# tud-amr/multi-robot-fabrics

Hardware: NVIDIA B200
Metric: fabric robot-steps/sec (3 Panda RF-CV) (higher is better)
Workload: dtype f32

## Files before the change

### __graft_entry__.py

```python
from __future__ import annotations

import os
import subprocess
import sys

ROOT = os.path.dirname(os.path.abspath(__file__))
PKG = os.path.join(ROOT, "multi-robot-fabrics_b200")
NVCC_FLAGS = ["-gencode", "arch=compute_100a,code=sm_100a", "-lineinfo", "-O3", "-std=c++17",
              "-Xcompiler", "-fPIC", "-shared"]


def _newer(target: str, sources) -> bool:
    if not os.path.exists(target):
        return False
    t = os.path.getmtime(target)
    return all(os.path.getmtime(s) <= t for s in sources)


def build(force: bool = False) -> None:
    csrc = os.path.join(PKG, "csrc")
    srcs = [os.path.join(csrc, f) for f in ("mrf_b200.cu", "mrf_device.cuh", "mrf_devcfg.h", "mrf_coop.cuh")]
    srcs.append(os.path.join(ROOT, "include", "mrf_b200.h"))
    so = os.path.join(PKG, "libmrf_b200.so")
    if force or not _newer(so, srcs):
        nvcc = os.environ.get("NVCC", "nvcc")
        subprocess.check_call([nvcc, *NVCC_FLAGS, "-o", so, srcs[0]])
    subprocess.check_call(["make", "-C", os.path.join(ROOT, "oracle"), "-s"])
    emul_so = os.path.join(ROOT, "tests", "emul", "libmrf_emul.so")
    emul_src = os.path.join(ROOT, "tests", "emul", "mrf_emul.cpp")
    if force or not _newer(emul_so, srcs[1:] + [emul_src]):
        subprocess.check_call(["g++", "-O2", "-std=c++17", "-fPIC", "-shared", "-ffp-contract=off", "-o", emul_so,
                               emul_src])
    if ROOT not in sys.path:
        sys.path.insert(0, ROOT)
    _probe_reference()
    import multi_robot_fabrics_b200 as m

    m._lib.lib()
    for name in m._lib.EXPORTS:
        getattr(m._lib.lib(), name)


_PROBED = False


def _probe_reference() -> None:
    global _PROBED
    if _PROBED:
        return
    _PROBED = True
    import importlib.util
    ref = os.path.join(ROOT, "baseline", "_ref")
    if os.path.isdir(ref) and ref not in sys.path:
        sys.path.append(ref)
    spec = importlib.util.spec_from_file_location("make_reference_golden",
                                                  os.path.join(ROOT, "tests", "golden", "make_reference_golden.py"))
    mod = importlib.util.module_from_spec(spec)
    spec.loader.exec_module(mod)
    ok, msg = mod.probe()
    gold = os.path.join(ROOT, "tests", "golden", "reference_golden.npz")
    state = "present" if os.path.exists(gold) else "absent"
    if ok:
        print(f"[build] reference dependencies available ({msg}); reference_golden.npz {state} -- "
              f"`python tests/golden/make_reference_golden.py` (re)generates it", file=sys.stderr)
    else:
        print(f"[build] reference dependencies {msg}: fabric arithmetic stays parity-unpinned "
              f"(baseline/_ref {'exists' if os.path.isdir(ref) else 'does not exist'}; reference_golden.npz {state})", file=sys.stderr)


def smoke() -> None:
    if ROOT not in sys.path:
        sys.path.insert(0, ROOT)
    import numpy as np
    import torch

    import multi_robot_fabrics_b200 as m
    from multi_robot_fabrics_b200.api import Fabrics, to_soa
    from oracle import o2
    from oracle.deadlock_ref import DeadlockOracle

    R, N, dev = 3, 20, "cuda:0"
    fab = Fabrics(R, device=0, estimate_goal=1, dl_dist_endeff=1.0)
    ocfg = o2.default_config(R)

    rec = m.scenarios.generate(64, R, seed=123)
# ... 80 lines not shown
```

### multi-robot-fabrics_b200/csrc/mrf_b200.cu

```cuda
#include <cuda_runtime.h>

#include <cmath>
#include <cstdio>
#include <cstdlib>
#include <cstring>
#include <new>
#include <string>
#include <vector>

#include "../../include/mrf_b200.h"
#include "mrf_device.cuh"
#include "mrf_devcfg.h"
#include "mrf_coop.cuh"

namespace mrf {

struct DlCfg {
    long long g_sr, g_sc, w_sr;
    int est_robot;
    int R, time_wait, time_gate;
    double avg_vel_constant, dist_constant, w_follower, w_leader, goal_scale, dist_endeff, backoff;
};

__device__ __forceinline__ double np_norm3(double x, double y, double z) {
// ... 281 lines not shown
            const unsigned t = atomicAdd(&sync[0], 1u);
            while (*reinterpret_cast<volatile unsigned*>(&sync[1]) + window <= t) __nanosleep(100);
            *tk = t;
        }
        __syncthreads();
        tile = *tk;
    }
    const long long b = (long long)tile * kTile + lane;
    const bool live = b < Bn;
    const long long bb = live ? b : Bn - 1;
    const T* ld_base = rec + (long long)r * B + bb;
    long long ld_stride = (long long)R * B;
    const T* tail = rec_tail;
    if (AOS) {
        const long long first = (long long)tile * kTile;
        const int nb = (int)(B - first < kTile ? B - first : kTile);
        const int nvals = nb * R * n_var;
        const int nvec = nvals * (int)sizeof(T) / 16;
        const T* srcT = rec + first * R * n_var;
        const int4* src = reinterpret_cast<const int4*>(srcT);
        int4* dst = reinterpret_cast<int4*>(kin);
        for (int i = tid; i < nvec; i += NT) dst[i] = src[i];
        for (int i = nvec * (16 / (int)sizeof(T)) + tid; i < nvals; i += NT) kin[i] = srcT[i];
        __syncthreads();
        if (tid == 0) atomicAdd(&sync[1], 1u);
        ld_base = kin + ((live ? lane : nb - 1) * R + r) * n_var;
        ld_stride = 1;
        tail += r * MRF_REC;
    }
    const long long b_src = STRIDE ? (long long)ex.list[bb] : 0;
    auto ld = [&](int f) {
        if (STRIDE)
            return f < ex.src_nvar ? (T)ex.src[f * ex.sf + r * ex.sr + b_src * ex.sb] : (T)ex.src_tail[r * MRF_REC + f];
        return AOS ? (f < n_var ? ld_base[f] : tail[f]) : rec[((long long)f * R + r) * B + bb];
    };
    (void)ld_stride;

    T q[kDof], qd[kDof];
#pragma unroll
    for (int i = 0; i < kDof; ++i) {
        q[i] = ld(MRF_Q + i);
        qd[i] = ld(MRF_QD + i);
    }
    load_params<T>(ld, prm, NT, tid);
    T* st_sph = prm + P_N * NT;
    if (!UNIFORM && !AOS && n_static > 0) {
        for (int i = 0; i < 4 * n_static; ++i) st_sph[i * NT + tid] = ex.stat[((long long)i * R + r) * B + bb];
    }
    if (AOS && ex.rec_out != nullptr && live) {
        for (int f = 0; f < n_var; ++f) ex.rec_out[((long long)f * R + r) * B + b] = ld_base[f];
    }
    Chain<T> ch;
    const T vref = cfg.static_or_dyn ? T(1) : T(0), aref = cfg.static_or_dyn ? cfg.sref : T(0);
    T acc = T(0);
    prm[P_RISK * NT + tid] = T(0);
    const bool want_pre = x_ee != nullptr || goal_est != nullptr || cfg.estimate_goal != 0;
    for (int k = want_pre ? -1 : 0; k < N; ++k) {
        if (k >= 0) {
#pragma unroll
            for (int i = 0; i < kDof; ++i) q[i] += cfg.dt * qd[i];
        }
        MRF_STEP_SYNC();
        chain_forward(cfg, r, q, qd, ch, kin, NT, tid);
        if (k < 0) {
            V3<T> p8 = kin_load(kin, NT, tid, 4, 0);
            if (x_ee != nullptr && live) {
                T* o = rec_order_out ? x_ee + (b * R + r) * 3 : x_ee + (long long)r * 3 * B + b;
                const long long st = rec_order_out ? 1 : B;
                o[0] = p8.x;
                o[st] = p8.y;
                o[2 * st] = p8.z;
            }
            if (r == cfg.estimate_robot) {
                V3<T> g = mk(prm[(P_G0 + 0) * NT + tid], prm[(P_G0 + 1) * NT + tid], prm[(P_G0 + 2) * NT + tid]);
                if (cfg.estimate_goal) {
                    V3<T> l1 = mk(cfg.link1[r][0], cfg.link1[r][1], cfg.link1[r][2]);
                    V3<T> v = cfg.estimate_goal == 1 ? cross(ch.z[0], p8 - l1) : kin_load(kin, NT, tid, 4, 3);
                    g = p8 + v * cfg.est_h;
                    prm[(P_G0 + 0) * NT + tid] = g.x;
                    prm[(P_G0 + 1) * NT + tid] = g.y;
                    prm[(P_G0 + 2) * NT + tid] = g.z;
                }
                if (goal_est != nullptr && live) {
                    T* o = rec_order_out ? goal_est + b * 3 : goal_est + b;
                    const long long st = rec_order_out ? 1 : B;
                    o[0] = g.x;
                    o[st] = g.y;
                    o[2 * st] = g.z;
                }
            }
            continue;
        }
        MRF_STEP_SYNC();
        T act[kDof], stiff;
        if (UNIFORM) {
            SmemSrcUniform<T, R> src{kin, lane, r, vref, aref, cfg.r_obst};
            fabric_action(cfg, r, q, qd, ch, kin, prm, NT, tid, src, act, &stiff);
        } else {
            SmemSrc<T> src{cfg, kin, NT, lane, r, vref, aref, st_sph, AOS ? 0 : n_static, tid};
            fabric_action(cfg, r, q, qd, ch, kin, prm, NT, tid, src, act, &stiff);
        }
        prm[P_RISK * NT + tid] = Mth<T>::max(prm[P_RISK * NT + tid], stiff);
#pragma unroll
        for (int i = 0; i < kDof; ++i) {
            qd[i] = act[i];
            acc += act[i] * act[i];
        }
        if (qN != nullptr && live) {
#pragma unroll
            for (int i = 0; i < kDof; ++i) qN[(((long long)r * N + k) * kDof + i) * B + b] = q[i];
        }
        if (qdN != nullptr && live) {
#pragma unroll
            for (int i = 0; i < kDof; ++i) qdN[(((long long)r * N + k) * kDof + i) * B + b] = qd[i];
        }
    }
    if (avg_vel != nullptr && live) avg_vel[rec_order_out ? b * R + r : (long long)r * B + b] = acc / (T(N) * T(kDof));
    if (risk != nullptr && live) risk[rec_order_out ? b * R + r : (long long)r * B + b] = prm[P_RISK * NT + tid];
    if (STRIDE) {
        __syncthreads();
        if (fused_post && tid < kTile && live)
            deadlock_one<float>(ex.dl.c, (long long)ex.list[b], ex.dl.B, (int)b, ex.dl.ov, ex.dl.x_ee, ex.dl.goals, ex.dl.weights,
                                ex.dl.avg_vel, nullptr, ex.dl.sm_state, ex.dl.time_step, ex.dl.tdo, ex.dl.st_int, ex.dl.st_goal,
                                ex.dl.flag, ex.dl.goal_est, ex.dl.result);
        tile_first += gridDim.x;
    }
    has_work = STRIDE && (long long)tile_first * kTile < Bn;
  }
    if (fused_post) {
        __syncthreads();
        if (threadIdx.x == 0) {
            __threadfence();
            if (atomicAdd(ex.dl.done, 1u) == gridDim.x - 1) {
                *ex.dl.done = 0;
                n_live[0] = 0;
            }
        }
    }
}

constexpr int kActThreads = 128;

#ifndef MRF_ACTION_MINBLOCKS
#define MRF_ACTION_MINBLOCKS 1
#endif
template <typename T, bool CART>
__global__ void __launch_bounds__(kActThreads, sizeof(T) == 4 ? MRF_ACTION_MINBLOCKS : 1)
    action_kernel(const __grid_constant__ DevCfg<T> cfg, int robot_first, int n_rob, const T* __restrict__ rec, int S,
                  const T* __restrict__ obst, int N, T* __restrict__ out, T* __restrict__ qN, T* __restrict__ qdN,
                  long long B, const int32_t* __restrict__ sm_state) {
// ... 615 lines not shown
extern "C" int mrf_set_coop_max_batch(mrf_handle_t h, int64_t max_batch) {
    if (!h || max_batch < 0) return fail(MRF_EINVAL, "mrf_set_coop_max_batch: bad argument");
    h->coop_max_batch = max_batch;
    return MRF_OK;
}
extern "C" int64_t mrf_launch_count(mrf_handle_t h) { return h ? h->launches : 0; }
extern "C" double mrf_last_kernel_ms(mrf_handle_t h) { return h ? h->last_ms : 0.0; }

template <typename T> static const DevCfg<T>& devcfg(mrf_handle_t h);
template <> const DevCfg<float>& devcfg<float>(mrf_handle_t h) { return h->c32; }
template <> const DevCfg<double>& devcfg<double>(mrf_handle_t h) { return h->c64; }

template <typename K> static int set_smem(K kernel, size_t bytes) {
    if (bytes > 48 * 1024) MRF_CUDA(cudaFuncSetAttribute(kernel, cudaFuncAttributeMaxDynamicSharedMemorySize, (int)bytes));
    return MRF_OK;
}
template <typename K> static void same_carveout(K kernel) {
#ifndef MRF_NO_CARVEOUT
    cudaFuncSetAttribute(kernel, cudaFuncAttributePreferredSharedMemoryCarveout, cudaSharedmemCarveoutMaxShared);
#endif
}

template <typename T>
static int rollout_dev(mrf_handle_t h, const T* rec, int N, T* avg_vel, T* x_ee, T* goal_est, T* qN, T* qdN, int64_t B,
                       void* stream, bool aos = false, int sync_slot = 0, int n_var = MRF_REC, const T* rec_tail = nullptr,
                       T* risk = nullptr, RollExtra<T> ex = RollExtra<T>{}) {
    unsigned* const n_live = ex.n_live;
    const int n_static = ex.n_static;
    const T* const stat = ex.stat;
    if (!h || (!rec && !n_live)) return fail(MRF_EINVAL, "mrf_rollout: null argument");
    if (B <= 0 || N <= 0) return fail(MRF_EINVAL, "mrf_rollout: B and N must be positive");
    MRF_CUDA(cudaSetDevice(h->device));
    const int R = h->cfg.n_robots, NT = kTile * R;
    if (aos && (qN || qdN)) return fail(MRF_EINVAL, "mrf_rollout: record-order input has no trajectory output");
    if (n_static < 0 || n_static > MRF_MAX_STATIC || (n_static > 0 && (!stat || aos || n_live)))
        return fail(MRF_EINVAL, "mrf_rollout: bad static-obstacle arguments");
    if (!aos && R >= 2 && B <= h->coop_max_batch && !risk && !n_live && n_static == 0) {
        switch (R) {
            case 2: rollout_coop_kernel<T, 2><<<(unsigned)B, 64, 0, (cudaStream_t)stream>>>(devcfg<T>(h), rec, N, avg_vel, x_ee, goal_est, qN, qdN, (long long)B); break;
            case 3: rollout_coop_kernel<T, 3><<<(unsigned)B, 96, 0, (cudaStream_t)stream>>>(devcfg<T>(h), rec, N, avg_vel, x_ee, goal_est, qN, qdN, (long long)B); break;
            case 4: rollout_coop_kernel<T, 4><<<(unsigned)B, 128, 0, (cudaStream_t)stream>>>(devcfg<T>(h), rec, N, avg_vel, x_ee, goal_est, qN, qdN, (long long)B); break;
            default: return fail(MRF_EINVAL, "mrf_rollout: n_robots out of range");
        }
        MRF_CUDA(cudaGetLastError());
        h->launches += 1;
        return MRF_OK;
    }
    const size_t smem = sizeof(T) * (size_t)(kKinRows<T> + P_N + 4 * n_static) * NT;
    long long grid = (B + kTile - 1) / kTile;
    if (n_live != nullptr && grid > 16) grid = 16;
    int rc = MRF_OK;
#define MRF_LAUNCH_ROLLOUT_K(RR, UU, AA, SS)                                                                         \
    {                                                                                                                \
        rc = set_smem(rollout_kernel<T, RR, UU, AA, SS>, smem);                                                      \
        same_carveout(rollout_kernel<T, RR, UU, AA, SS>);                                                            \
        if (rc) return rc;                                                                                           \
        rollout_kernel<T, RR, UU, AA, SS><<<(unsigned)grid, NT, smem, (cudaStream_t)stream>>>(                       \
            devcfg<T>(h), rec, N, avg_vel, x_ee, goal_est, qN, qdN, (long long)B, h->d_sync + 2 * sync_slot,        \
            (unsigned)h->zc_window, n_var, rec_tail, risk, ex);                                                      \
    }
#define MRF_LAUNCH_ROLLOUT(RR)                                                                                       \
    case RR:                                                                                                         \
        if (devcfg<T>(h).uniform_obst && n_static == 0) {                                                            \
            if (aos) MRF_LAUNCH_ROLLOUT_K(RR, true, true, false)                                                     \
            else if (stride) MRF_LAUNCH_ROLLOUT_STRIDE(RR, true)                                                     \
            else MRF_LAUNCH_ROLLOUT_K(RR, true, false, false)                                                        \
        } else {                                                                                                     \
            if (aos) MRF_LAUNCH_ROLLOUT_K(RR, false, true, false)                                                    \
            else if (stride) MRF_LAUNCH_ROLLOUT_STRIDE(RR, false)                                                    \
            else MRF_LAUNCH_ROLLOUT_K(RR, false, false, false)                                                       \
        }                                                                                                            \
        break;
#define MRF_LAUNCH_ROLLOUT_STRIDE(RR, UU)                                                                            \
    {                                                                                                                \
        if constexpr (sizeof(T) == 8) MRF_LAUNCH_ROLLOUT_K(RR, UU, false, true)                                      \
        else return fail(MRF_EINVAL, "mrf_rollout: device-side count is FP64 only");                                 \
    }
    const bool stride = n_live != nullptr;
    if (aos) MRF_CUDA(cudaMemsetAsync(h->d_sync + 2 * sync_slot, 0, 2 * sizeof(unsigned), (cudaStream_t)stream));
    switch (R) {
        MRF_LAUNCH_ROLLOUT(1)
        MRF_LAUNCH_ROLLOUT(2)
        MRF_LAUNCH_ROLLOUT(3)
        MRF_LAUNCH_ROLLOUT(4)
        default: return fail(MRF_EINVAL, "mrf_rollout: n_robots out of range");
    }
#undef MRF_LAUNCH_ROLLOUT_STRIDE
#undef MRF_LAUNCH_ROLLOUT_K
#undef MRF_LAUNCH_ROLLOUT
    MRF_CUDA(cudaGetLastError());
    h->launches += 1;
    return MRF_OK;
}

template <typename T, bool CART>
static int action_dev(mrf_handle_t h, int robot_first, int n_rob, const T* rec, int S, const T* obst, int N, T* out,
                      T* qN, T* qdN, int64_t B, void* stream, const int32_t* sm_state = nullptr) {
    if (!h || !rec || (S > 0 && !obst)) return fail(MRF_EINVAL, "mrf_action: null argument");
    if (B <= 0 || S < 0 || n_rob < 1 || robot_first < 0 || robot_first + n_rob > h->cfg.n_robots)
        return fail(MRF_EINVAL, "mrf_action: bad sizes");
    if (CART && N <= 0) return fail(MRF_EINVAL, "mrf_rollout_cart: needs N > 0");
    MRF_CUDA(cudaSetDevice(h->device));
    static const int env_thr = getenv("MRF_ACTION_THREADS_F64") ? atoi(getenv("MRF_ACTION_THREADS_F64")) : 32;
    const int threads = sizeof(T) == 8 ? env_thr : kActThreads;
    const size_t smem = sizeof(T) * (size_t)(kKinRows<T> + P_N + kObstRing * MRF_OBST) * threads;
    int rc = set_smem(action_kernel<T, CART>, smem);
    if (rc) return rc;
    const long long total = (long long)n_rob * B;
    const long long grid = (total + threads - 1) / threads;
    action_kernel<T, CART><<<(unsigned)grid, threads, smem, (cudaStream_t)stream>>>(
// ... 1274 lines not shown
```

### multi-robot-fabrics_b200/csrc/mrf_device.cuh

```cuda
#pragma once

#include <stdint.h>

#if defined(__CUDACC__)
#define MRF_HD __host__ __device__ __forceinline__
#else
#define MRF_HD inline
#include <cmath>
#endif

#include "../../include/mrf_b200.h"

namespace mrf {

template <int N> struct Int {
    static constexpr int value = N;
};

constexpr int kDof = 7;
constexpr int kEgo = 5;
constexpr int kPts = kEgo + 1;
constexpr int kZ = kPts * 9;
#ifdef MRF_AXES_SMEM_F32
template <typename T> constexpr bool kAxesInSmem = true;
// ... 419 lines not shown
    V3<P2<T>> b;
    V3<P2<T>> nv;
};
template <typename T> MRF_HD void acc2_zero(PointAcc2<T>& a) {
    const P2<T> z = psplat(T(0));
    a.A = Sym3<P2<T>>{z, z, z, z, z, z};
    a.b = V3<P2<T>>{z, z, z};
    a.nv = V3<P2<T>>{z, z, z};
}
template <typename T, bool IRHO>
MRF_HD void sphere_leaf2(const V3<P2<T>>& p, const V3<P2<T>>& v, const V3<P2<T>>& cc, const V3<P2<T>>& xo,
                         const V3<P2<T>>& vo, const V3<P2<T>>& co, T vref, T aref, P2<T> rho, P2<T> irho, P2<T> cM, T sigma,
                         PointAcc2<T>& acc) {
    const P2<T> m1 = psplat(T(-1)), nvref = psplat(-vref);
    V3<P2<T>> d{pfma(xo.x, m1, p.x), pfma(xo.y, m1, p.y), pfma(xo.z, m1, p.z)};
    V3<P2<T>> w{pfma(vo.x, nvref, v.x), pfma(vo.y, nvref, v.y), pfma(vo.z, nvref, v.z)};
    P2<T> n2 = pdot(d, d);
    P2<T> in1 = prsqrt(n2);
    P2<T> gs, ix, nrin;
    if (IRHO) {
        gs = pmul(in1, irho);
        ix = prcp(pfma(n2, gs, m1));
        nrin = pmul(in1, rho);
    } else {
        P2<T> n = pmul(n2, in1);
        P2<T> t = pfma(rho, m1, n);
        P2<T> nr = pmul(n, rho);
        P2<T> u = prcp(pmul(nr, t));
        gs = pmul(u, t);
        ix = pmul(pmul(u, nr), rho);
        nrin = pmul(pmul(in1, rho), m1);
    }
    P2<T> dw = pdot(d, w), da = pdot(d, co);
    P2<T> wc = pfma(d.z, cc.z, pfma(d.y, cc.y, pfma(d.x, cc.x, pdot(w, w))));
    P2<T> ix2 = pmul(ix, ix), ix4 = pmul(ix2, ix2);
    P2<T> Ml = pmul(cM, ix4);
    P2<T> Mg = pmul(Ml, gs);
    P2<T> k = pmul(Mg, gs);
    P2<T> u1 = pmul(k, pmul(dw, dw));
    P2<T> hh = pmul(ix4, psplat(T(-0.5)));
    P2<T> fl = pmul(u1, hh);
    P2<T> fd = pmul(u1, pfma(ix, psplat(T(2)), hh));
    P2<T> X = pfma(u1, nrin, pmul(Mg, wc));
    P2<T> fq = pfma(X, psplat(sigma), pfma(pmul(Mg, da), psplat(-aref), fl));
    P2<T> ge = pmul(gs, pfma(X, psplat(sigma - T(1)), fd));
    acc.nv.x = pfma(d.x, ge, acc.nv.x); acc.nv.y = pfma(d.y, ge, acc.nv.y); acc.nv.z = pfma(d.z, ge, acc.nv.z);
    V3<P2<T>> Md{pmul(d.x, k), pmul(d.y, k), pmul(d.z, k)};
    acc.A.xx = pfma(Md.x, d.x, acc.A.xx); acc.A.xy = pfma(Md.x, d.y, acc.A.xy); acc.A.xz = pfma(Md.x, d.z, acc.A.xz);
    acc.A.yy = pfma(Md.y, d.y, acc.A.yy); acc.A.yz = pfma(Md.y, d.z, acc.A.yz); acc.A.zz = pfma(Md.z, d.z, acc.A.zz);
    P2<T> gf = pmul(gs, fq);
    acc.b.x = pfma(d.x, gf, acc.b.x); acc.b.y = pfma(d.y, gf, acc.b.y); acc.b.z = pfma(d.z, gf, acc.b.z);
}

template <typename T>
MRF_HD void plane_leaf(V3<T> p, V3<T> v, V3<T> cc, V3<T> nh, T dn, T rb, T wt, T sigma, PointAcc<T>& acc, T& num) {
    T x = dot(nh, p) + dn - rb;
    T xd = dot(nh, v);
    T s = xd > T(0) ? T(0) : (xd < T(0) ? T(1) : T(0.5));
    T ix = Mth<T>::rcp(x);
    T xd2 = xd * xd;
    T Ml = ((T(0.2) * wt) * s) * ix * ix;
    T u = Ml * xd2;
    T h = T(-10) * xd2 * Mth<T>::rcp(T(1) + Mth<T>::exp(T(10) * x));
    T fl = Ml * h;
    T X = Ml * dot(nh, cc);
    T fq = fl + sigma * X;
    num += xd * ((fl + u * ix) + (sigma - T(1)) * X);
    V3<T> Mg = nh * Ml;
    acc.A.xx += Mg.x * nh.x; acc.A.xy += Mg.x * nh.y; acc.A.xz += Mg.x * nh.z;
    acc.A.yy += Mg.y * nh.y; acc.A.yz += Mg.y * nh.z; acc.A.zz += Mg.z * nh.z;
    acc.b = acc.b + nh * fq;
}

template <typename T, int K, typename Org>
MRF_HD void jac_cols(const Chain<T>& ch, const T* kin, int NT, int tid, V3<T> p, const Org& org, V3<T>* Jc) {
#pragma unroll
    for (int j = 0; j < K; ++j) Jc[j] = cross(axis_of(ch, kin, NT, tid, j), p - org(j));
}

template <typename T, int K> MRF_HD void pullback(const V3<T>* Jc, const PointAcc<T>& acc, Spec<T>& S) {
#pragma unroll
    for (int j = 0; j < K; ++j) {
        V3<T> AJ = symmul(acc.A, Jc[j]);
        S.f[j] += dot(Jc[j], acc.b);
#pragma unroll
        for (int i = 0; i <= j; ++i) S.M[i][j] += dot(Jc[i], AJ);
    }
}

template <typename T> MRF_HD void chol_solve6(T (&M)[6][6], T eps, const T* b, T* x) {
    T inv[6];
#pragma unroll
    for (int j = 0; j < 6; ++j) {
        T s = M[j][j] + eps;
#pragma unroll
        for (int k = 0; k < j; ++k) s -= M[k][j] * M[k][j];
        T r = Mth<T>::rsqrt(s);
        inv[j] = r;
        M[j][j] = s * r;
#pragma unroll
        for (int i = j + 1; i < 6; ++i) {
            T t = M[j][i];
#pragma unroll
            for (int k = 0; k < j; ++k) t -= M[k][j] * M[k][i];
            M[j][i] = t * r;
        }
// ... 75 lines not shown
        for (int k = 0; k < i; ++k) s += N[k][i] * y[k];
        y[i] = s * inv[i];
    }
#pragma unroll
    for (int i = 5; i >= 0; --i) {
        T s = y[i];
#pragma unroll
        for (int k = i + 1; k < 6; ++k) s += N[i][k] * x[k];
        x[i] = s * inv[i];
    }
}
template <typename T> MRF_HD void chol_solve6n_pair(P2<T> (&N)[6][6], T eps, const P2<T>* b, P2<T>* x) {
    P2<T> inv[6];
    const P2<T> ne = psplat(-eps);
#pragma unroll
    for (int j = 0; j < 6; ++j) {
        P2<T> s = padd(N[j][j], ne);
#pragma unroll
        for (int k = 0; k < j; ++k) s = pfma(N[k][j], N[k][j], s);
        P2<T> r = pmk(Mth<T>::rsqrt(-plo(s)), Mth<T>::rsqrt(-phi(s)));
        inv[j] = r;
#pragma unroll
        for (int i = j + 1; i < 6; ++i) {
            P2<T> t = N[j][i];
#pragma unroll
            for (int k = 0; k < j; ++k) t = pfma(N[k][j], N[k][i], t);
            N[j][i] = pmul(t, r);
        }
    }
    P2<T> y[6];
#pragma unroll
    for (int i = 0; i < 6; ++i) {
        P2<T> s = b[i];
#pragma unroll
        for (int k = 0; k < i; ++k) s = pfma(N[k][i], y[k], s);
        y[i] = pmul(s, inv[i]);
    }
#pragma unroll
    for (int i = 5; i >= 0; --i) {
        P2<T> s = y[i];
#pragma unroll
        for (int k = i + 1; k < 6; ++k) s = pfma(N[i][k], x[k], s);
        x[i] = pmul(s, inv[i]);
    }
}

template <typename T> MRF_HD void attractor_scalars(T n, T w, T& dpsi, T& m2) {
    dpsi = T(5) * w * Mth<T>::tanh(T(10) * n);
    m2 = T(2) * (T(1.7) * Mth<T>::exp(T(-0.5625) * n * n) + T(0.3));
}

template <typename T, typename Src>
MRF_HD void fabric_action(const DevCfg<T>& cfg, int r, const T* q, const T* qd, const Chain<T>& ch, const T* kin,
                          const T* prm, int NT, int tid, const Src& src, T* act, T* stiff = nullptr) {
    const T sigma = cfg.sigma;
    T stiff_sum = T(0);
    Spec<T> G;
#pragma unroll
    for (int i = 0; i < 6; ++i) {
#pragma unroll
        for (int j = 0; j < 6; ++j) G.M[i][j] = T(0);
        G.M[i][i] = T(-0.2);
        G.f[i] = T(0);
    }
    G.m7 = T(0.2);
    G.f[6] = T(0);
    T num = T(0);

#pragma unroll
    for (int i = 0; i < kDof; ++i) {
        const P2<T> x2 = pmk(q[i] - cfg.lim[i][0], cfg.lim[i][1] - q[i]);
        const T sl = qd[i] > T(0) ? T(0) : (qd[i] < T(0) ? T(1) : T(0.5));
        const P2<T> ix = prcp(x2);
        const P2<T> t = pmul(pmk(sl, T(1) - sl), ix);
        const P2<T> u = pmul(pmul(psplat(qd[i] * qd[i]), ix), t);
        const T Ml = T(0.2) * (plo(t) + phi(t));
        if (i < 6) G.M[i][i] -= Ml; else G.m7 += Ml;
        const T du = plo(u) - phi(u);
        G.f[i] += T(-0.02) * du;
        num += qd[i] * (T(0.08) * du);
    }


    V3<T> org_[6];
    if (!kAxesInSmem<T>) {
        org_[0] = mk(cfg.link1[r][0], cfg.link1[r][1], cfg.link1[r][2]);
        org_[1] = org_[0];
        org_[2] = kin_load(kin, NT, tid, 0, 0);
        org_[3] = kin_load(kin, NT, tid, 1, 0);
        org_[4] = kin_load(kin, NT, tid, 2, 0);
        org_[5] = org_[4];
    }
    auto org = [&](int j) -> V3<T> {
        if (!kAxesInSmem<T>) return org_[j];
        return j < 2 ? mk(cfg.link1[r][0], cfg.link1[r][1], cfg.link1[r][2]) : kin_load(kin, NT, tid, j < 4 ? j - 2 : 2, 0);
    };

    constexpr bool kKeepJ8 = sizeof(T) == 4;
    V3<T> Jc[6];
    bool have_j8 = false;
    if (src.collide(cfg.has_coll != 0)) {
        const V3<T> nh = mk(prm[(P_NH + 0) * NT + tid], prm[(P_NH + 1) * NT + tid], prm[(P_NH + 2) * NT + tid]);
        const T dn = prm[P_DN * NT + tid];
        constexpr bool kObstMajor = Src::kObstacleMajor && sizeof(T) == 4;
        int em = 0x3F;
        if constexpr (!Src::kFullLinks) em = cfg.ego_mask[r];
        PointAcc2<T> om[3];
        if (kObstMajor) {
            V3<P2<T>> pp[3], vv[3], cp[3];
            P2<T> rbp[3];
#pragma unroll
            for (int ps = 0; ps < 3; ++ps) {
                const int ea = ps == 0 ? 0 : (ps == 1 ? 2 : 3), eb = ps == 0 ? 1 : (ps == 1 ? 2 : 4);
                V3<T> pa = kin_load(kin, NT, tid, ea, 0), pb = kin_load(kin, NT, tid, eb, 0);
                V3<T> va = kin_load(kin, NT, tid, ea, 3), vb = kin_load(kin, NT, tid, eb, 3);
                V3<T> ca = kin_load(kin, NT, tid, ea, 6), cb = kin_load(kin, NT, tid, eb, 6);
                pp[ps] = V3<P2<T>>{pmk(pa.x, pb.x), pmk(pa.y, pb.y), pmk(pa.z, pb.z)};
                vv[ps] = V3<P2<T>>{pmk(va.x, vb.x), pmk(va.y, vb.y), pmk(va.z, vb.z)};
                cp[ps] = V3<P2<T>>{pmk(ca.x, cb.x), pmk(ca.y, cb.y), pmk(ca.z, cb.z)};
                rbp[ps] = pmk(prm[(P_RB + 2 * ps) * NT + tid], prm[(P_RB + 2 * ps + 1) * NT + tid]);
// ... 45 lines not shown
        }
#pragma unroll 1
        for (int e = 0; e < kEgo; ++e) {
            const int K = e < 3 ? e + 2 : 6;
            const int rb_first = e + (e > 2 ? 1 : 0);
            V3<T> p = kin_load(kin, NT, tid, e, 0), v = kin_load(kin, NT, tid, e, 3), cc = kin_load(kin, NT, tid, e, 6);
            PointAcc<T> acc;
            acc.A = Sym3<T>{T(0), T(0), T(0), T(0), T(0), T(0)};
            acc.b = mk(T(0), T(0), T(0));
            T rb = prm[(P_RB + rb_first) * NT + tid];
            T we = T(1);
            int passes = 1;
            if (e == 2) {
                T rb2 = prm[(P_RB + rb_first + 1) * NT + tid];
                if (Src::kFullLinks || ((em >> rb_first) & 3) == 3) {
                    if (rb2 == rb) we = T(2); else passes = 2;
                } else if ((em >> (rb_first + 1)) & 1) {
                    rb = rb2;
                } else if (!((em >> rb_first) & 1)) {
                    passes = 0;
                }
            } else if (!Src::kFullLinks && !((em >> rb_first) & 1)) {
                passes = 0;
            }
            if (!Src::kFullLinks && passes == 0) continue;
            if (kObstMajor) {
                auto pick = [&](const P2<T>& s0, const P2<T>& s1, const P2<T>& s2) {
                    return e == 0 ? plo(s0) : e == 1 ? phi(s0) : e == 2 ? plo(s1) + phi(s1) : e == 3 ? plo(s2) : phi(s2);
                };
                acc.A.xx = pick(om[0].A.xx, om[1].A.xx, om[2].A.xx); acc.A.xy = pick(om[0].A.xy, om[1].A.xy, om[2].A.xy);
                acc.A.xz = pick(om[0].A.xz, om[1].A.xz, om[2].A.xz); acc.A.yy = pick(om[0].A.yy, om[1].A.yy, om[2].A.yy);
                acc.A.yz = pick(om[0].A.yz, om[1].A.yz, om[2].A.yz); acc.A.zz = pick(om[0].A.zz, om[1].A.zz, om[2].A.zz);
                acc.b.x = pick(om[0].b.x, om[1].b.x, om[2].b.x); acc.b.y = pick(om[0].b.y, om[1].b.y, om[2].b.y);
                acc.b.z = pick(om[0].b.z, om[1].b.z, om[2].b.z);
                num += dot(v, mk(pick(om[0].nv.x, om[1].nv.x, om[2].nv.x), pick(om[0].nv.y, om[1].nv.y, om[2].nv.y),
                                 pick(om[0].nv.z, om[1].nv.z, om[2].nv.z)));
            }
            if (kObstMajorD) {
                auto pk = [&](T a0, T a1, T a2, T a3, T a4) { return e == 0 ? a0 : e == 1 ? a1 : e == 2 ? a2 : e == 3 ? a3 : a4; };
                acc.A.xx = pk(od[0].A.xx, od[1].A.xx, od[2].A.xx, od[3].A.xx, od[4].A.xx);
                acc.A.xy = pk(od[0].A.xy, od[1].A.xy, od[2].A.xy, od[3].A.xy, od[4].A.xy);
                acc.A.xz = pk(od[0].A.xz, od[1].A.xz, od[2].A.xz, od[3].A.xz, od[4].A.xz);
                acc.A.yy = pk(od[0].A.yy, od[1].A.yy, od[2].A.yy, od[3].A.yy, od[4].A.yy);
                acc.A.yz = pk(od[0].A.yz, od[1].A.yz, od[2].A.yz, od[3].A.yz, od[4].A.yz);
                acc.A.zz = pk(od[0].A.zz, od[1].A.zz, od[2].A.zz, od[3].A.zz, od[4].A.zz);
                acc.b.x = pk(od[0].b.x, od[1].b.x, od[2].b.x, od[3].b.x, od[4].b.x);
                acc.b.y = pk(od[0].b.y, od[1].b.y, od[2].b.y, od[3].b.y, od[4].b.y);
                acc.b.z = pk(od[0].b.z, od[1].b.z, od[2].b.z, od[3].b.z, od[4].b.z);
            }
            constexpr bool kPackedSpheres = sizeof(T) == 4 && !kObstMajor;
            const T rb0 = rb;
            for (int pass = 0; pass < passes; ++pass) {
                if (pass == 1) rb = prm[(P_RB + rb_first + 1) * NT + tid];
                if (!kPackedSpheres && !kObstMajor && !kObstMajorD) {
                    if constexpr (Src::kUniformRadius) {
                        const T rho = src.ro + rb, irho = Mth<T>::rcp(rho);
                        src.each([&](V3<T> xo, V3<T> vo, V3<T> co, T, T wo) {
                            sphere_leaf<T, true>(p, v, cc, xo, vo, co, src.vref, src.aref, rho, we * wo, sigma, acc, num, irho);
                        });
                    } else {
                        src.each([&](V3<T> xo, V3<T> vo, V3<T> co, T ro, T wo) {
                            sphere_leaf(p, v, cc, xo, vo, co, src.vref, src.aref, ro + rb, we * wo, sigma, acc, num);
                        });
                    }
                }
                if constexpr (Src::kHasStatic)
                    src.each_static([&](V3<T> xo, T ro) {
                        const V3<T> z0 = mk(T(0), T(0), T(0));
                        sphere_leaf(p, v, cc, xo, z0, z0, T(0), T(0), ro + rb, we, sigma, acc, num);
                    });
                plane_leaf(p, v, cc, nh, dn, rb, we, sigma, acc, num);
            }
            if (kPackedSpheres) {
                PointAcc2<T> acc2;
                acc2.A = Sym3<P2<T>>{pmk(acc.A.xx, T(0)), pmk(acc.A.xy, T(0)), pmk(acc.A.xz, T(0)),
                                     pmk(acc.A.yy, T(0)), pmk(acc.A.yz, T(0)), pmk(acc.A.zz, T(0))};
                acc2.b = V3<P2<T>>{pmk(acc.b.x, T(0)), pmk(acc.b.y, T(0)), pmk(acc.b.z, T(0))};
                acc2.nv = V3<P2<T>>{psplat(T(0)), psplat(T(0)), psplat(T(0))};
                const V3<P2<T>> p2{psplat(p.x), psplat(p.y), psplat(p.z)}, v2{psplat(v.x), psplat(v.y), psplat(v.z)},
                    c2{psplat(cc.x), psplat(cc.y), psplat(cc.z)};
                const P2<T> cw = psplat(T(0.02) * we);
                rb = rb0;
                for (int pass = 0; pass < passes; ++pass) {
                    if (pass == 1) rb = prm[(P_RB + rb_first + 1) * NT + tid];
                    if constexpr (Src::kUniformRadius) {
                        const P2<T> irho = psplat(Mth<T>::rcp(src.ro + rb)), nrho = psplat(-(src.ro + rb));
                        src.each2([&](const V3<P2<T>>& xo, const V3<P2<T>>& vo, const V3<P2<T>>& co, P2<T>, P2<T> wo) {
                            sphere_leaf2<T, true>(p2, v2, c2, xo, vo, co, src.vref, src.aref, nrho, irho, pmul(wo, cw), sigma, acc2);
                        });
                    } else {
                        src.each2([&](const V3<P2<T>>& xo, const V3<P2<T>>& vo, const V3<P2<T>>& co, P2<T> ro, P2<T> wo) {
                            sphere_leaf2<T, false>(p2, v2, c2, xo, vo, co, src.vref, src.aref, padd(ro, psplat(rb)), ro,
                                                   pmul(wo, cw), sigma, acc2);
                        });
                    }
                }
                acc.A.xx = plo(acc2.A.xx) + phi(acc2.A.xx); acc.A.xy = plo(acc2.A.xy) + phi(acc2.A.xy);
                acc.A.xz = plo(acc2.A.xz) + phi(acc2.A.xz); acc.A.yy = plo(acc2.A.yy) + phi(acc2.A.yy);
                acc.A.yz = plo(acc2.A.yz) + phi(acc2.A.yz); acc.A.zz = plo(acc2.A.zz) + phi(acc2.A.zz);
                acc.b.x = plo(acc2.b.x) + phi(acc2.b.x); acc.b.y = plo(acc2.b.y) + phi(acc2.b.y);
                acc.b.z = plo(acc2.b.z) + phi(acc2.b.z);
                num = Mth<T>::fma(v.x, plo(acc2.nv.x) + phi(acc2.nv.x),
                                  Mth<T>::fma(v.y, plo(acc2.nv.y) + phi(acc2.nv.y), Mth<T>::fma(v.z, plo(acc2.nv.z) + phi(acc2.nv.z), num)));
            }
            stiff_sum += (acc.A.xx + acc.A.yy) + acc.A.zz;
            if (kKeepJ8 && e == kEgo - 1) have_j8 = true;
#pragma unroll
            for (int j = 0; j < 6; ++j)
                if (j < K) Jc[j] = cross(axis_of(ch, kin, NT, tid, j), p - org(j));
#pragma unroll
            for (int j = 0; j < 6; ++j) {
                if (j < K) {
                    V3<T> AJ = symmul(acc.A, Jc[j]);
                    G.f[j] = dot_add(Jc[j], acc.b, G.f[j]);
#pragma unroll
                    for (int i = 0; i <= j; ++i) G.M[i][j] = dot_sub(Jc[i], AJ, G.M[i][j]);
                }
            }
        }
    }

    if (stiff != nullptr) *stiff = stiff_sum;

    T qMq = G.m7 * qd[6] * qd[6];
#pragma unroll
    for (int i = 0; i < 6; ++i) {
// ... 45 lines not shown
            F.f[j] = dot_add(Jc[j], t0, dot_add(Jd[j], u1, F.f[j]));
#pragma unroll
            for (int i = 0; i <= j; ++i) F.M[i][j] = dot_add(Jc[i], A0, dot_add(Jd[i], A1, F.M[i][j]));
        }
        T x2 = q[6] - prm[P_G2 * NT + tid];
        T dpsi2, m2;
        attractor_scalars(Mth<T>::abs(x2), prm[P_W2 * NT + tid], dpsi2, m2);
        F.f[6] += m2 * dpsi2 * (x2 > T(0) ? T(1) : (x2 < T(0) ? T(-1) : T(0)));
        F.m7 += m2;
    }

    T hg[kDof], hf[kDof];
    if (sizeof(T) == 4) {
        P2<T> M2[6][6], b2[6], x2[6];
#pragma unroll
        for (int j = 0; j < 6; ++j) {
            b2[j] = pmk(G.f[j], F.f[j]);
#pragma unroll
            for (int i = 0; i <= j; ++i) M2[i][j] = pmk(G.M[i][j], F.M[i][j]);
        }
        chol_solve6n_pair(M2, e, b2, x2);
#pragma unroll
        for (int j = 0; j < 6; ++j) {
            hg[j] = plo(x2[j]);
            hf[j] = phi(x2[j]);
        }
    } else {
        chol_solve6n(G.M, e, G.f, hg);
        chol_solve6n(F.M, e, F.f, hf);
    }
    hg[6] = G.f[6] * Mth<T>::rcp(G.m7 + e);
    hf[6] = F.f[6] * Mth<T>::rcp(F.m7 + e);
    T qq = T(0), qhg = T(0), qhf = T(0);
#pragma unroll
    for (int i = 0; i < kDof; ++i) {
        qq += qd[i] * qd[i];
        qhg += qd[i] * hg[i];
        qhf += qd[i] * hf[i];
    }
    const T iden = Mth<T>::rcp(e + cfg.s2 * qq);
    const T a_ex0 = -cfg.s2 * qhg * iden, a_exf = -cfg.s2 * qhf * iden;
    const T eta = T(0.5) * (Mth<T>::tanh(T(-0.45) * qq - T(0.5)) + T(1));
    const T a_ex = eta * a_ex0 + (T(1) - eta) * a_exf;
    const T beta = T(0.5) * (Mth<T>::tanh(T(-0.5) * (xpsi - T(0.02))) + T(1)) * T(6.5) + T(0.01) +
                   Mth<T>::max(T(0), a_geom - a_ex);
    const T damp = a_ex + beta;
#pragma unroll
    for (int i = 0; i < kDof; ++i) {
        T qdd = -hf[i] - damp * qd[i];
        act[i] = cfg.mode == 1 ? qd[i] + cfg.dt * qdd : qdd;
    }
}

constexpr int kTile = 32;

template <typename T> struct SmemSrc {
    static constexpr bool kUniformRadius = false;
    static constexpr bool kFullLinks = false;
    static constexpr bool kHasStatic = true;
    template <typename F> MRF_HD void each_static(F f) const {
        for (int o = 0; o < n_static; ++o) {
            const T* b = stat + (o * 4) * NT + tid_s;
            f(mk(b[0], b[NT], b[2 * NT]), b[3 * NT]);
        }
    }
    static constexpr bool kObstacleMajor = false;
    MRF_HD bool collide(bool has) const { return has; }
    const DevCfg<T>& cfg;
    const T* kin;
    int NT, lane, r;
    T vref, aref;
    const T* stat = nullptr;
    int n_static = 0, tid_s = 0;
    template <typename F> MRF_HD void each(F f) const {
        const int ne = cfg.ent_n[r];
#pragma unroll 2
        for (int k = 0; k < ne; ++k) {
            const int t = cfg.ent_rob[r][k] * kTile + lane, e = cfg.ent_src[r][k];
            f(kin_load(kin, NT, t, e, 0), kin_load(kin, NT, t, e, 3), kin_load(kin, NT, t, e, 6), cfg.ent_rad[r][k],
              cfg.ent_w[r][k]);
        }
    }
    template <typename F> MRF_HD void each2(F f) const {
        const int ne = cfg.ent_n[r];
        for (int k = 0; k < ne; k += 2) {
            const int k1 = k + 1 < ne ? k + 1 : k;
            const int ta = cfg.ent_rob[r][k] * kTile + lane, tb = cfg.ent_rob[r][k1] * kTile + lane;
            const int ea = cfg.ent_src[r][k], eb = cfg.ent_src[r][k1];
            const V3<T> xa = kin_load(kin, NT, ta, ea, 0), va = kin_load(kin, NT, ta, ea, 3), ca = kin_load(kin, NT, ta, ea, 6);
            const V3<T> xb = kin_load(kin, NT, tb, eb, 0), vb = kin_load(kin, NT, tb, eb, 3), cb = kin_load(kin, NT, tb, eb, 6);
            f(V3<P2<T>>{pmk(xa.x, xb.x), pmk(xa.y, xb.y), pmk(xa.z, xb.z)},
              V3<P2<T>>{pmk(va.x, vb.x), pmk(va.y, vb.y), pmk(va.z, vb.z)},
              V3<P2<T>>{pmk(ca.x, cb.x), pmk(ca.y, cb.y), pmk(ca.z, cb.z)},
              pmk(cfg.ent_rad[r][k], cfg.ent_rad[r][k1]), pmk(cfg.ent_w[r][k], k1 == k ? T(0) : cfg.ent_w[r][k1]));
        }
    }
};

template <typename T, int R> struct SmemSrcUniform {
    static constexpr bool kUniformRadius = true;
    static constexpr bool kFullLinks = true;
    static constexpr bool kHasStatic = false;
    static constexpr bool kObstacleMajor = false;
    MRF_HD bool collide(bool has) const { return has; }
    const T* kin;
    int lane, r;
    T vref, aref, ro;
    template <typename F> MRF_HD void each(F f) const {
// ... 153 lines not shown
```

Before: 3.897 billion.

## Share pairwise sphere-leaf terms between robot pairs via shared memory

```diff
diff --git a/__graft_entry__.py b/__graft_entry__.py
--- a/__graft_entry__.py
+++ b/__graft_entry__.py
@@ -26,11 +26,12 @@
         nvcc = os.environ.get("NVCC", "nvcc")
         subprocess.check_call([nvcc, *NVCC_FLAGS, "-o", so, srcs[0]])
     subprocess.check_call(["make", "-C", os.path.join(ROOT, "oracle"), "-s"])
-    emul_so = os.path.join(ROOT, "tests", "emul", "libmrf_emul.so")
-    emul_src = os.path.join(ROOT, "tests", "emul", "mrf_emul.cpp")
-    if force or not _newer(emul_so, srcs[1:] + [emul_src]):
-        subprocess.check_call(["g++", "-O2", "-std=c++17", "-fPIC", "-shared", "-ffp-contract=off", "-o", emul_so,
-                               emul_src])
+    for name in ("mrf_emul", "mrf_emul_pair"):
+        emul_so = os.path.join(ROOT, "tests", "emul", f"lib{name}.so")
+        emul_src = os.path.join(ROOT, "tests", "emul", f"{name}.cpp")
+        if force or not _newer(emul_so, srcs[1:] + [emul_src]):
+            subprocess.check_call(["g++", "-O2", "-std=c++17", "-fPIC", "-shared", "-ffp-contract=off", "-o", emul_so,
+                                   emul_src])
     if ROOT not in sys.path:
         sys.path.insert(0, ROOT)
     _probe_reference()
diff --git a/multi-robot-fabrics_b200/csrc/mrf_b200.cu b/multi-robot-fabrics_b200/csrc/mrf_b200.cu
--- a/multi-robot-fabrics_b200/csrc/mrf_b200.cu
+++ b/multi-robot-fabrics_b200/csrc/mrf_b200.cu
@@ -357,6 +357,14 @@
     }
     Chain<T> ch;
     const T vref = cfg.static_or_dyn ? T(1) : T(0), aref = cfg.static_or_dyn ? cfg.sref : T(0);
+    constexpr bool kPair = kPairPath<T, R, UNIFORM>;
+    const bool pair_cfg = kPair && pair_leaves_cfg(cfg);
+    bool pair_on = false;
+    T* const pls = prm + P_N * NT;
+    if (pair_cfg) {
+        __syncthreads();
+        pair_on = pair_leaves_lane(prm, NT, lane);
+    }
     T acc = T(0);
     prm[P_RISK * NT + tid] = T(0);
     const bool want_pre = x_ee != nullptr || goal_est != nullptr || cfg.estimate_goal != 0;
@@ -400,7 +408,13 @@
         T act[kDof], stiff;
         if (UNIFORM) {
             SmemSrcUniform<T, R> src{kin, lane, r, vref, aref, cfg.r_obst};
-            fabric_action(cfg, r, q, qd, ch, kin, prm, NT, tid, src, act, &stiff);
+            PairLeaves<T> pl{T(0), pair_on};
+            if (pair_cfg) {
+                if (pair_on) pl.num = pair_leaves_eval(cfg, r, kin, prm, pls, NT, tid, lane);
+                __syncthreads();
+                if (pair_on) pl.num += pls[2 * kPairSlots * NT + (r == 0 ? 2 : r - 1) * kTile + lane];
+            }
+            fabric_action(cfg, r, q, qd, ch, kin, prm, NT, tid, src, act, &stiff, kPair ? &pl : nullptr);
         } else {
             SmemSrc<T> src{cfg, kin, NT, lane, r, vref, aref, st_sph, AOS ? 0 : n_static, tid};
             fabric_action(cfg, r, q, qd, ch, kin, prm, NT, tid, src, act, &stiff);
@@ -1122,10 +1136,11 @@
     int rc = MRF_OK;
 #define MRF_LAUNCH_ROLLOUT_K(RR, UU, AA, SS)                                                                         \
     {                                                                                                                \
-        rc = set_smem(rollout_kernel<T, RR, UU, AA, SS>, smem);                                                      \
+        const size_t smem_k = smem + (kPairPath<T, RR, UU> ? sizeof(T) * (size_t)kPairRows * NT : 0);               \
+        rc = set_smem(rollout_kernel<T, RR, UU, AA, SS>, smem_k);                                                    \
         same_carveout(rollout_kernel<T, RR, UU, AA, SS>);                                                            \
         if (rc) return rc;                                                                                           \
-        rollout_kernel<T, RR, UU, AA, SS><<<(unsigned)grid, NT, smem, (cudaStream_t)stream>>>(                       \
+        rollout_kernel<T, RR, UU, AA, SS><<<(unsigned)grid, NT, smem_k, (cudaStream_t)stream>>>(                     \
             devcfg<T>(h), rec, N, avg_vel, x_ee, goal_est, qN, qdN, (long long)B, h->d_sync + 2 * sync_slot,        \
             (unsigned)h->zc_window, n_var, rec_tail, risk, ex);                                                      \
     }
diff --git a/multi-robot-fabrics_b200/csrc/mrf_device.cuh b/multi-robot-fabrics_b200/csrc/mrf_device.cuh
--- a/multi-robot-fabrics_b200/csrc/mrf_device.cuh
+++ b/multi-robot-fabrics_b200/csrc/mrf_device.cuh
@@ -495,6 +495,153 @@
     acc.b.x = pfma(d.x, gf, acc.b.x); acc.b.y = pfma(d.y, gf, acc.b.y); acc.b.z = pfma(d.z, gf, acc.b.z);
 }
 
+#ifdef MRF_NO_PAIR_LEAVES
+constexpr bool kPairLeaves = false;
+#else
+constexpr bool kPairLeaves = true;
+#endif
+constexpr int kTile = 32;
+constexpr int kPairSlots = kEgo * (kPts / 2) * 2;
+constexpr int kPairRows = 2 * kPairSlots + 1;
+template <typename T, int R, bool UNIFORM> constexpr bool kPairPath = kPairLeaves && UNIFORM && R == 3 && sizeof(T) == 4;
+
+MRF_HD void pl_put(float* pl, int NT, int t, int s, P2<float> x) { reinterpret_cast<float2*>(pl)[s * NT + t] = x.v; }
+MRF_HD void pl_put(double* pl, int NT, int t, int s, P2<double> x) {
+    pl[(s * NT + t) * 2] = x.a;
+    pl[(s * NT + t) * 2 + 1] = x.b;
+}
+MRF_HD P2<float> pl_get(const float* pl, int NT, int t, int s) { return P2<float>{reinterpret_cast<const float2*>(pl)[s * NT + t]}; }
+MRF_HD P2<double> pl_get(const double* pl, int NT, int t, int s) { return pmk(pl[(s * NT + t) * 2], pl[(s * NT + t) * 2 + 1]); }
+template <typename T> MRF_HD T pl_half(const T* pl, int NT, int t, int s, int h) { return pl[(s * NT + t) * 2 + h]; }
+
+template <typename T> struct PairLeaves {
+    T num;
+    bool on;
+};
+
+template <typename T> MRF_HD bool pair_leaves_cfg(const DevCfg<T>& cfg) {
+    return cfg.n_robots == 3 && cfg.uniform_obst != 0 && cfg.has_coll != 0 && cfg.static_or_dyn != 0 && cfg.sigma == cfg.sref;
+}
+template <typename T> MRF_HD bool pair_leaves_lane(const T* prm, int NT, int lane) {
+    const T r0 = prm[P_RB * NT + lane];
+    bool eq = true;
+    for (int j = 0; j < 3; ++j)
+#pragma unroll
+        for (int l = 0; l < 6; ++l) eq = eq && prm[(P_RB + l) * NT + j * kTile + lane] == r0;
+    return eq;
+}
+
+template <typename T>
+MRF_HD void sphere_leaf2_shared(const V3<P2<T>>& p, const V3<P2<T>>& v, const V3<P2<T>>& cc, const V3<P2<T>>& xo,
+                                const V3<P2<T>>& vo, const V3<P2<T>>& co, P2<T> nrho, P2<T> irho, P2<T> cM, T sigma,
+                                P2<T>& k, P2<T>& gf, V3<P2<T>>& nv, P2<T>& nvb) {
+    const P2<T> m1 = psplat(T(-1));
+    V3<P2<T>> d{pfma(xo.x, m1, p.x), pfma(xo.y, m1, p.y), pfma(xo.z, m1, p.z)};
+    V3<P2<T>> w{pfma(vo.x, m1, v.x), pfma(vo.y, m1, v.y), pfma(vo.z, m1, v.z)};
+    P2<T> n2 = pdot(d, d);
+    P2<T> in1 = prsqrt(n2);
+    P2<T> gs = pmul(in1, irho);
+    P2<T> ix = prcp(pfma(n2, gs, m1));
+    P2<T> nrin = pmul(in1, nrho);
+    P2<T> dw = pdot(d, w), da = pdot(d, co);
+    P2<T> ww = pdot(w, w);
+    P2<T> wc = pfma(d.z, cc.z, pfma(d.y, cc.y, pfma(d.x, cc.x, ww)));
+    P2<T> wcb = pfma(da, m1, ww);
+    P2<T> ix2 = pmul(ix, ix), ix4 = pmul(ix2, ix2);
+    P2<T> Ml = pmul(cM, ix4);
+    P2<T> Mg = pmul(Ml, gs);
+    k = pmul(Mg, gs);
+    P2<T> u1 = pmul(k, pmul(dw, dw));
+    P2<T> hh = pmul(ix4, psplat(T(-0.5)));
+    P2<T> fl = pmul(u1, hh);
+    P2<T> fd = pmul(u1, pfma(ix, psplat(T(2)), hh));
+    P2<T> X = pfma(u1, nrin, pmul(Mg, wc));
+    P2<T> Xb = pfma(u1, nrin, pmul(Mg, wcb));
+    P2<T> fq = pfma(X, psplat(sigma), pfma(pmul(Mg, da), psplat(-sigma), fl));
+    const P2<T> s1 = psplat(sigma - T(1));
+    P2<T> ge = pmul(gs, pfma(X, s1, fd));
+    nv.x = pfma(d.x, ge, nv.x); nv.y = pfma(d.y, ge, nv.y); nv.z = pfma(d.z, ge, nv.z);
+    P2<T> geb = pmul(gs, pfma(Xb, s1, fd));
+    nvb = pfma(pdot(d, vo), geb, nvb);
+    gf = pmul(gs, fq);
+}
+
+template <typename T>
+MRF_HD T pair_leaves_eval(const DevCfg<T>& cfg, int r, const T* kin, const T* prm, T* pl, int NT, int tid, int lane) {
+    const int t = (r == 2 ? 0 : r + 1) * kTile + lane;
+    const T rho = cfg.r_obst + prm[P_RB * NT + tid];
+    const P2<T> irho = psplat(Mth<T>::rcp(rho)), nrho = psplat(-rho);
+    T num = T(0);
+    P2<T> nvb = psplat(T(0));
+#pragma unroll 1
+    for (int e = 0; e < kEgo; ++e) {
+        const V3<T> p = kin_load(kin, NT, tid, e, 0), v = kin_load(kin, NT, tid, e, 3), cc = kin_load(kin, NT, tid, e, 6);
+        const V3<P2<T>> p2{psplat(p.x), psplat(p.y), psplat(p.z)}, v2{psplat(v.x), psplat(v.y), psplat(v.z)},
+            c2{psplat(cc.x), psplat(cc.y), psplat(cc.z)};
+        const T cw = T(0.02) * (e == 2 ? T(2) : T(1));
+        V3<P2<T>> nv{psplat(T(0)), psplat(T(0)), psplat(T(0))};
+#pragma unroll
+        for (int pp = 0; pp < kPts / 2; ++pp) {
+            P2<T> k, gf;
+            sphere_leaf2_shared(p2, v2, c2, kin_load_pair(kin, NT, t, pp, 0), kin_load_pair(kin, NT, t, pp, 3),
+                                kin_load_pair(kin, NT, t, pp, 6), nrho, irho,
+                                pmk(pp == 1 ? T(2) * cw : cw, pp == 2 ? T(2) * cw : cw), cfg.sigma, k, gf, nv, nvb);
+            pl_put(pl, NT, tid, (e * 3 + pp) * 2, k);
+            pl_put(pl, NT, tid, (e * 3 + pp) * 2 + 1, gf);
+        }
+        num = Mth<T>::fma(v.x, plo(nv.x) + phi(nv.x),
+                          Mth<T>::fma(v.y, plo(nv.y) + phi(nv.y), Mth<T>::fma(v.z, plo(nv.z) + phi(nv.z), num)));
+    }
+    pl[2 * kPairSlots * NT + tid] = -(plo(nvb) + phi(nvb));
+    return num;
+}
+
+template <typename T>
+MRF_HD void pair_leaves_rebuild(const DevCfg<T>& cfg, int r, const T* kin, const T* pl, int NT, int tid, int lane, int e,
+                                V3<T> p, V3<T> v, V3<T> cc, T rb, T we, PointAcc<T>& acc, T& num) {
+    const int tn = (r == 2 ? 0 : r + 1) * kTile + lane, tp = (r == 0 ? 2 : r - 1) * kTile + lane;
+    const V3<P2<T>> x2p = kin_load_pair(kin, NT, tp, 2, 0);
+    const T rho = cfg.r_obst + rb;
+    const V3<T> z0 = mk(T(0), T(0), T(0));
+    sphere_leaf<T, true>(p, v, cc, mk(phi(x2p.x), phi(x2p.y), phi(x2p.z)), z0, z0, T(0), T(0), rho, T(2) * we, cfg.sigma,
+                         acc, num, Mth<T>::rcp(rho));
+    const int pe = e >> 1, he = e & 1;
+    {
+        const V3<T> d = p - mk(plo(x2p.x), plo(x2p.y), plo(x2p.z));
+        const int s = (4 * 3 + pe) * 2;
+        const T k = pl_half(pl, NT, tp, s, he), gf = pl_half(pl, NT, tp, s + 1, he);
+        const V3<T> Md = d * k;
+        acc.A.xx = Mth<T>::fma(Md.x, d.x, acc.A.xx); acc.A.xy = Mth<T>::fma(Md.x, d.y, acc.A.xy);
+        acc.A.xz = Mth<T>::fma(Md.x, d.z, acc.A.xz); acc.A.yy = Mth<T>::fma(Md.y, d.y, acc.A.yy);
+        acc.A.yz = Mth<T>::fma(Md.y, d.z, acc.A.yz); acc.A.zz = Mth<T>::fma(Md.z, d.z, acc.A.zz);
+        acc.b.x = Mth<T>::fma(d.x, gf, acc.b.x); acc.b.y = Mth<T>::fma(d.y, gf, acc.b.y); acc.b.z = Mth<T>::fma(d.z, gf, acc.b.z);
+    }
+    const P2<T> m1 = psplat(T(-1));
+    Sym3<P2<T>> A{pmk(acc.A.xx, T(0)), pmk(acc.A.xy, T(0)), pmk(acc.A.xz, T(0)), pmk(acc.A.yy, T(0)), pmk(acc.A.yz, T(0)),
+                  pmk(acc.A.zz, T(0))};
+    V3<P2<T>> b{pmk(acc.b.x, T(0)), pmk(acc.b.y, T(0)), pmk(acc.b.z, T(0))};
+    const V3<P2<T>> p2{psplat(p.x), psplat(p.y), psplat(p.z)};
+    auto add = [&](const V3<P2<T>>& xo, P2<T> k, P2<T> gf) {
+        const V3<P2<T>> d{pfma(xo.x, m1, p2.x), pfma(xo.y, m1, p2.y), pfma(xo.z, m1, p2.z)};
+        const V3<P2<T>> Md{pmul(d.x, k), pmul(d.y, k), pmul(d.z, k)};
+        A.xx = pfma(Md.x, d.x, A.xx); A.xy = pfma(Md.x, d.y, A.xy); A.xz = pfma(Md.x, d.z, A.xz);
+        A.yy = pfma(Md.y, d.y, A.yy); A.yz = pfma(Md.y, d.z, A.yz); A.zz = pfma(Md.z, d.z, A.zz);
+        b.x = pfma(d.x, gf, b.x); b.y = pfma(d.y, gf, b.y); b.z = pfma(d.z, gf, b.z);
+    };
+#pragma unroll
+    for (int pp = 0; pp < kPts / 2; ++pp)
+        add(kin_load_pair(kin, NT, tn, pp, 0), pl_get(pl, NT, tid, (e * 3 + pp) * 2), pl_get(pl, NT, tid, (e * 3 + pp) * 2 + 1));
+#pragma unroll
+    for (int pp = 0; pp < 2; ++pp) {
+        const int s0 = ((2 * pp) * 3 + pe) * 2, s1 = ((2 * pp + 1) * 3 + pe) * 2;
+        add(kin_load_pair(kin, NT, tp, pp, 0), pmk(pl_half(pl, NT, tp, s0, he), pl_half(pl, NT, tp, s1, he)),
+            pmk(pl_half(pl, NT, tp, s0 + 1, he), pl_half(pl, NT, tp, s1 + 1, he)));
+    }
+    acc.A.xx = plo(A.xx) + phi(A.xx); acc.A.xy = plo(A.xy) + phi(A.xy); acc.A.xz = plo(A.xz) + phi(A.xz);
+    acc.A.yy = plo(A.yy) + phi(A.yy); acc.A.yz = plo(A.yz) + phi(A.yz); acc.A.zz = plo(A.zz) + phi(A.zz);
+    acc.b.x = plo(b.x) + phi(b.x); acc.b.y = plo(b.y) + phi(b.y); acc.b.z = plo(b.z) + phi(b.z);
+}
+
 template <typename T>
 MRF_HD void plane_leaf(V3<T> p, V3<T> v, V3<T> cc, V3<T> nh, T dn, T rb, T wt, T sigma, PointAcc<T>& acc, T& num) {
     T x = dot(nh, p) + dn - rb;
@@ -676,8 +823,10 @@
 
 template <typename T, typename Src>
 MRF_HD void fabric_action(const DevCfg<T>& cfg, int r, const T* q, const T* qd, const Chain<T>& ch, const T* kin,
-                          const T* prm, int NT, int tid, const Src& src, T* act, T* stiff = nullptr) {
+                          const T* prm, int NT, int tid, const Src& src, T* act, T* stiff = nullptr,
+                          const PairLeaves<T>* pair = nullptr) {
     const T sigma = cfg.sigma;
+    const bool pair_on = kPairLeaves && Src::kUniformRadius && pair != nullptr && pair->on;
     T stiff_sum = T(0);
     Spec<T> G;
 #pragma unroll
@@ -689,7 +838,7 @@
     }
     G.m7 = T(0.2);
     G.f[6] = T(0);
-    T num = T(0);
+    T num = pair_on ? pair->num : T(0);
 
 #pragma unroll
     for (int i = 0; i < kDof; ++i) {
@@ -841,7 +990,7 @@
             const T rb0 = rb;
             for (int pass = 0; pass < passes; ++pass) {
                 if (pass == 1) rb = prm[(P_RB + rb_first + 1) * NT + tid];
-                if (!kPackedSpheres && !kObstMajor && !kObstMajorD) {
+                if (!kPackedSpheres && !kObstMajor && !kObstMajorD && !pair_on) {
                     if constexpr (Src::kUniformRadius) {
                         const T rho = src.ro + rb, irho = Mth<T>::rcp(rho);
                         src.each([&](V3<T> xo, V3<T> vo, V3<T> co, T, T wo) {
@@ -860,7 +1009,9 @@
                     });
                 plane_leaf(p, v, cc, nh, dn, rb, we, sigma, acc, num);
             }
-            if (kPackedSpheres) {
+            if (pair_on) {
+                pair_leaves_rebuild(cfg, r, kin, prm + P_N * NT, NT, tid, tid % kTile, e, p, v, cc, rb0, we, acc, num);
+            } else if (kPackedSpheres) {
                 PointAcc2<T> acc2;
                 acc2.A = Sym3<P2<T>>{pmk(acc.A.xx, T(0)), pmk(acc.A.xy, T(0)), pmk(acc.A.xz, T(0)),
                                      pmk(acc.A.yy, T(0)), pmk(acc.A.yz, T(0)), pmk(acc.A.zz, T(0))};
@@ -1012,8 +1163,6 @@
     }
 }
 
-constexpr int kTile = 32;
-
 template <typename T> struct SmemSrc {
     static constexpr bool kUniformRadius = false;
     static constexpr bool kFullLinks = false;
```

Result: faster. 4.102 billion (median of 6 runs) (+5.3%).
